# oscarkey/safe-exploration

Measured on AMD Instinct MI355X. Metric: cem_particle_step_evals_per_s, higher is better.
Workload: dtype f64

## Files before the change

### include/sx_amd.h

```cpp
#ifndef SX_AMD_H
#define SX_AMD_H

#include <stdint.h>

#ifdef __cplusplus
extern "C" {
#endif

#define SX_MAX_NS 4
#define SX_MAX_NU 2
#define SX_MAX_D (SX_MAX_NS + SX_MAX_NU)
#define SX_MAX_M 16
#define SX_TILE 16

#define SX_OK 0
#define SX_ERR_ARG 1
#define SX_ERR_UNSUPPORTED 2
#define SX_ERR_LAUNCH 3

#define SX_STATUS_NAN 1
#define SX_STATUS_ZERO_FIX 2
#define SX_STATUS_UB_NONPOS 4

#define SX_OBJ_NEG_VARIANCE 0
// ... 350 lines not shown
int sx_cem_rollout_cons_multi(const sx_gp_model* models, const void* table, const sx_env* env, const sx_con_set* cons,
                              const sx_sat_cost* cost, int E, int P, int H, const double* x0, const double* q0,
                              const double* mean, const double* std, const double* noise, double* actions, double* traj,
                              double* sigma, double* obj_cost, double* con_cost, int32_t* status, void* stream);
int sx_cem_rollout_elites_cons_multi(const sx_gp_model* models, const void* table, const sx_env* env, const sx_con_set* cons,
                                     const sx_sat_cost* cost, int E, int P, int H, const double* x0, const double* q0,
                                     const double* elite_rows, int k, const double* noise, double* actions, double* traj,
                                     double* sigma, double* obj_cost, double* con_cost, int32_t* status, double* mean_out,
                                     double* std_out, void* stream);
int sx_cem_rollout_cons_multi_form(const sx_gp_model* models, int E, int H);

int sx_cem_rollout_starts_cons(const sx_gp_model* model, const sx_env* env, const sx_con_set* cons, int E, int P, int H,
                               const double* mean, const double* std, const double* noise, double* rows, double* traj,
                               double* sigma, double* obj_cost, double* con_cost, int32_t* status, void* stream);

int sx_cem_rollout_starts_multi(const sx_gp_model* models, const void* table, const sx_env* env, int E, int P, int H,
                                const double* mean, const double* std, const double* noise, double* rows, double* traj,
                                double* sigma, double* obj_cost, double* con_cost, int32_t* status , void* stream);
int sx_cem_rollout_starts_cons_multi(const sx_gp_model* models, const void* table, const sx_env* env,
                                     const sx_con_set* cons, int E, int P, int H, const double* mean, const double* std,
                                     const double* noise, double* rows, double* traj, double* sigma, double* obj_cost,
                                     double* con_cost, int32_t* status , void* stream);
int sx_cem_rollout_starts_multi_form(const sx_gp_model* models, int E, int H);

int sx_cem_pack_result(int G, int E, int row_len, const int32_t* status, const int32_t* best_ok, const double* q_block,
                       int64_t q_count, const double* best, double* out, void* stream);

int sx_cem_rank_counts(int E, int P);

int sx_cem_rank_refit(int E, int P, int k, int row_len, const double* con_cost, const double* obj_cost,
                      int64_t cost_stride, const double* actions, int64_t act_stride, int32_t* elite_idx,
                      double* elite_rows, double* mean, double* std, double* best, int32_t* best_ok, void* stream);

#ifdef __cplusplus
}
#endif
#endif
```

### safe_exploration_amd/_lib.py

```python
import ctypes
import os
from ctypes import POINTER, Structure, c_char_p, c_double, c_int, c_int32, c_int64, c_uint8, c_void_p

import numpy as np
import torch

SX_MAX_NS = 4
SX_MAX_NU = 2
SX_MAX_D = SX_MAX_NS + SX_MAX_NU
SX_MAX_M = 16
SX_SAT_MAX_DIM = SX_MAX_NS + 1
SX_TILE = 16
SX_GP_FIT_ENTRY_BYTES = 360
SX_GP_APPEND_ENTRY_BYTES = 408
SX_FEAT_MAX_WIDTH = 32
SX_FEAT_MAX_LAYERS = 3
SX_MLP_MAX_HIDDEN = 4
SX_MLP_MAX_WIDTH = 64

SX_OK, SX_ERR_ARG, SX_ERR_UNSUPPORTED, SX_ERR_LAUNCH = 0, 1, 2, 3
SX_STATUS_NAN, SX_STATUS_ZERO_FIX, SX_STATUS_UB_NONPOS, SX_STATUS_NOT_PD = 1, 2, 4, 8
SX_OBJ_NEG_VARIANCE, SX_OBJ_AFFINE_ABS = 0, 1
SX_CON_TERMINAL, SX_CON_ALL_STATES = 0, 1
SX_PROF_ROLLOUT_FUSED, SX_PROF_RANK, SX_PROF_KSTAR_BIG, SX_PROF_TRMM_BIG, SX_PROF_STEP_BIG, SX_PROF_ROLLOUT_FEAT, SX_PROF_ROLLOUT_MLP = range(7)
# ... 154 lines not shown
                                         c_int] + [c_void_p] * 12),
    'sx_cem_rollout_elites_sat_multi': (c_int, [POINTER(SxGpModel), c_void_p, POINTER(SxEnv), POINTER(SxSatCost), c_int,
                                                c_int, c_int, c_void_p, c_void_p, c_void_p, c_int] + [c_void_p] * 10),
    'sx_cem_rollout_sat_form': (c_int, [POINTER(SxGpModel), c_int]),
    'sx_conset_eval': (c_int, [POINTER(SxEnv), POINTER(SxConSet), c_int] + [c_void_p] * 4 + [c_int, c_void_p, c_void_p]),
    'sx_cem_rollout_cons': (c_int, [POINTER(SxGpModel), POINTER(SxEnv), POINTER(SxConSet), POINTER(SxSatCost), c_int, c_int,
                                    c_int] + [c_void_p] * 12),
    'sx_cem_rollout_elites_cons': (c_int, [POINTER(SxGpModel), POINTER(SxEnv), POINTER(SxConSet), POINTER(SxSatCost), c_int,
                                           c_int, c_int, c_void_p, c_void_p, c_void_p, c_int] + [c_void_p] * 10),
    'sx_cem_rollout_cons_form': (c_int, [POINTER(SxGpModel), c_int]),
    'sx_cem_rollout_cons_multi': (c_int, [POINTER(SxGpModel), c_void_p, POINTER(SxEnv), POINTER(SxConSet),
                                          POINTER(SxSatCost), c_int, c_int, c_int] + [c_void_p] * 12),
    'sx_cem_rollout_elites_cons_multi': (c_int, [POINTER(SxGpModel), c_void_p, POINTER(SxEnv), POINTER(SxConSet),
                                                 POINTER(SxSatCost), c_int, c_int, c_int, c_void_p, c_void_p, c_void_p,
                                                 c_int] + [c_void_p] * 10),
    'sx_cem_rollout_cons_multi_form': (c_int, [POINTER(SxGpModel), c_int, c_int]),
    'sx_cem_rollout_starts_cons': (c_int, [POINTER(SxGpModel), POINTER(SxEnv), POINTER(SxConSet), c_int, c_int, c_int]
                                   + [c_void_p] * 10),
    'sx_cem_rollout_starts_multi': (c_int, [POINTER(SxGpModel), c_void_p, POINTER(SxEnv), c_int, c_int, c_int]
                                    + [c_void_p] * 10),
    'sx_cem_rollout_starts_cons_multi': (c_int, [POINTER(SxGpModel), c_void_p, POINTER(SxEnv), POINTER(SxConSet), c_int,
                                                 c_int, c_int] + [c_void_p] * 10),
    'sx_cem_rollout_starts_multi_form': (c_int, [POINTER(SxGpModel), c_int, c_int]),
    'sx_profile_enable': (c_int, [c_int]),
    'sx_profile_stride': (c_int, [c_int]),
    'sx_profile_stride_kind': (c_int, [c_int, c_int]),
    'sx_profile_collect': (c_int, [c_int, POINTER(c_double), POINTER(c_int64)]),
    'sx_profile_disable': (c_int, []),
    'sx_cem_rank_counts': (c_int, [c_int, c_int]),
    'sx_cem_rollout_form': (c_int, [POINTER(SxGpModel), c_int]),
    'sx_cem_pack_result': (c_int, [c_int, c_int, c_int, c_void_p, c_void_p, c_void_p, c_int64, c_void_p, c_void_p, c_void_p]),
    'sx_cem_rank_refit': (c_int, [c_int, c_int, c_int, c_int, c_void_p, c_void_p, c_int64, c_void_p, c_int64]
                          + [c_void_p] * 7),
}

LIB_PATH = os.environ.get('SX_LIB') or os.path.join(os.path.dirname(os.path.abspath(__file__)), 'csrc', 'libsxamd.so')
_lib = None


class SxError(RuntimeError):
    pass


def lib():
    global _lib
    if _lib is None:
        if not os.path.exists(LIB_PATH):
            raise SxError(f'{LIB_PATH} is missing: build it with `python -c "import __graft_entry__ as g; g.build()"` '
                          f'(safe_exploration_amd has no CPU fallback)')
        handle = ctypes.CDLL(LIB_PATH)
        for name, (res, args) in SIGNATURES.items():
            fn = getattr(handle, name)
            fn.restype = res
            fn.argtypes = args
        _lib = handle
    return _lib


def check(code: int, what: str) -> None:
    if code != SX_OK:
        raise SxError(f'{what}: {_ERR.get(code, code)}')


def ptr(t):
    if t is None:
        return None
# ... 31 lines not shown
```

### safe_exploration_amd/cem_mpc.py

```python
import ctypes
from dataclasses import dataclass
from typing import List, NamedTuple, Optional, Sequence, Tuple

import torch
from torch import Tensor

from . import _lib, distributed
from .costs import SaturatingCost
from .gp_reachability_pytorch import raise_for_status, save_failure_state
from .ssm_cem.gp_ssm_cem import GpCemSSM


@dataclass
class Rollouts:
    trajectories: Optional[Tensor]
    actions: Tensor
    objective_costs: Tensor
    constraint_costs: Tensor
    perf_trajectories: Optional[Tensor] = None
    perf_sigma: Optional[Tensor] = None
    perf_cov: Optional[Tensor] = None


def _rollout(suffix: str, head: tuple, x0: Tensor, horizon: int, n_s: int, n_u: int, words: int, unsupported, *,
             actions, mean, std, noise, q0, want_traj, want_sigma, status, elite_rows, want_dist, workspace=()):
    dev = x0.device
    E = x0.size(0)
    if noise is not None:
        P = noise.size(1)
        actions = torch.empty((E, P, horizon, n_u), dtype=torch.float64, device=dev)
    else:
        P = actions.size(1)
        actions = actions.contiguous()
# ... 732 lines not shown
        raise ValueError(f'{share} particles per GPU rank in {chunks} chunks: num_elites={num_elites} is '
                         f'too large for it (limit {min(share // chunks, RANK_MAX_CANDIDATES // chunks)})')


def expand_init_std(init_std, horizon: int, n_u: int) -> Tensor:
    std = torch.as_tensor(init_std, dtype=torch.float64).cpu()
    return (std.reshape(horizon, -1) if std.dim() > 0 else std).expand(horizon, n_u).clone()


def cem_rank_refit_any(con: Tensor, obj: Tensor, actions: Tensor, k: int, **kw):
    E, P = con.shape
    C = rank_chunks(P)
    if C == 1:
        return cem_rank_refit(con, obj, actions, k, **kw)
    Pc, L = P // C, actions[0, 0].numel()
    if k > Pc or C * k > RANK_MAX_CANDIDATES:
        raise ValueError(f'{P} candidates rank in {C} chunks of {Pc}: k={k} must not exceed the chunk size, nor '
                         f'{C} k the kernel\'s {RANK_MAX_CANDIDATES}')
    local = cem_rank_refit(con.reshape(E * C, Pc), obj.reshape(E * C, Pc), actions.reshape(E * C, Pc, L), k,
                           want_rows=True, want_refit=False)
    flat = local['elite_rows'].reshape(-1)
    return cem_rank_refit(flat, flat[1:], flat[2:], k, cost_stride=2 + L, act_stride=2 + L, row_len=L,
                          num_candidates=C * k, num_problems=E, **kw)


def _hand_off(owner, best: Tensor, best_ok: Tensor, status: Tensor, q_block: Optional[Tensor]):
    G, E, L = status.numel(), best_ok.numel(), best[0].numel()
    n = G + E + 1 + E * L
    packed = torch.empty(n, dtype=torch.float64, device=best.device)
    _lib.check(_lib.lib().sx_cem_pack_result(G, E, L, _lib.ptr(status), _lib.ptr(best_ok), _lib.ptr(q_block),
                                             q_block.numel() if q_block is not None else 0,
                                             _lib.ptr(best.contiguous()), _lib.ptr(packed),
                                             _lib.stream_ptr(best.device)), 'sx_cem_pack_result')
    host = getattr(owner, '_pinned', None)
    if host is None or host.numel() < n:
        owner._pinned = host = torch.empty(max(n, 256), dtype=torch.float64).pin_memory()
    host[:n].copy_(packed, non_blocking=True)
    torch.cuda.current_stream(best.device).synchronize()
    out = host[:n].clone()
    return (out[:G].to(torch.int64), out[G:G + E] != 0, bool(out[G + E] != 0),
            out[G + E + 1:].view(best.shape))


def fold_status(words) -> int:
    out = 0
    for w in words.reshape(-1).tolist():
        out |= int(w)
    return out


def _cem_iterations(iterations: int, rollout, rank, mean: Tensor, std: Tensor):
    rows = out = None
    for it in range(iterations):
        out = rank(it, rollout(it, mean, std, rows))
        if out['mean'] is None:
            rows = out['elite_rows']
        else:
            mean, std = out['mean'].view(mean.shape), out['std'].view(std.shape)
    return out


def _check_solve(owner, x0: Tensor, q_block: Optional[Tensor], best: Tensor, best_ok: Tensor, status: Tensor, where: str,
                 problems):
    words, found, is_nonpoint, best_host = _hand_off(owner, best, best_ok, status, q_block)
    if is_nonpoint:
        raise NotImplementedError(f'{where} starts from point states (all-zero Q), as CemSafeMPC.get_action does')
    statuses = [fold_status(words[r]) for _, r in problems]
    both = _lib.SX_STATUS_NAN | _lib.SX_STATUS_ZERO_FIX
    repeated = False
    for i, (s, r) in enumerate(problems):
        if (statuses[i] & both) == both and owner._last_noise is not None:
            owner.stepwise_fallbacks += 1
            repeated = True
            b, ok, _, st = s.solve(x0[r], noise=owner._last_noise[:, r].contiguous(), stepwise=True)
            w, found[r], _, best_host[r] = _hand_off(owner, b, ok, st, None)
            statuses[i] = fold_status(w)
    for (s, _), st in zip(problems, statuses):
        s.last_status = st
    for i, ((s, r), st) in enumerate(zip(problems, statuses)):
        raise_for_status(st, where if len(problems) == 1 else f'{where} (problem {i})',
                         dump=lambda s=s, r=r: save_failure_state(s._ssm, x0[r], s._last_actions if s is owner else None))
    return best_host, found, repeated


def _checked_cost(cost, n_s: int, kind: Optional[str], on_safety: bool = False):
    if cost is None:
        return None
    if not isinstance(cost, SaturatingCost):
        raise TypeError(f'cost must be a costs.SaturatingCost or None, got {type(cost).__name__}')
    if kind != 'taylor' and not on_safety:
        raise ValueError("a SaturatingCost prices (mean, covariance) pairs: it needs a performance trajectory with "
                         "cem_perf_type='taylor' (perf_type='taylor', n_perf > 0), not "
                         + ('no performance trajectory' if kind is None else f'the {kind!r} form')
                         + ('; without one, cost_on_safety=True (cem_cost_on_safety) prices the safety ellipsoids'
                            if kind is None else ''))
    if cost.n_s != n_s:
        raise ValueError(f'the cost is built for n_s = {cost.n_s}, the model has n_s = {n_s}')
    return cost


class FusedCemMpc:

    def __init__(self, ssm: GpCemSSM, env: _lib.SxEnv, time_horizon: int, num_rollouts: int, num_elites: int,
                 num_iterations: int, *, device=None, seed: int = 0, init_std=1.0, warm_start: str = 'zero',
                 record_rollouts: bool = False, process_group=None, force_exchange: bool = False, n_perf: int = 0,
                 perf_r: int = 1, perf_variance: bool = False, perf_type: str = 'mean_equivalent',
                 perf_terminal_safety: bool = False, cost_on_safety: bool = False, con_set=None):
        self._ssm = ssm
        self._con_set = _checked_con_set(con_set, ssm)
        if con_set is not None:
            if int(n_perf) > 0:
                raise NotImplementedError(f'con_set constrains the safety trajectory of a solve without a performance '
                                          f'trajectory: got n_perf={n_perf} (cem_n_perf > 0 is not built)')
            if process_group is not None:
                raise NotImplementedError('con_set is not built for sharded particles (a process group)')
        self._cost_on_safety = bool(cost_on_safety)
        if self._cost_on_safety and int(n_perf) > 0:
            raise ValueError(f'cost_on_safety=True prices the safety trajectory, which carries the objective only without a '
                             f'performance trajectory: got n_perf={n_perf}.  The cost belongs to one trajectory, chosen by '
                             f"n_perf (n_perf > 0 with perf_type='taylor' prices the performance trajectory)")
        self._env = env
        self._horizon = time_horizon
        self._perf = PerfSpec(n_perf, perf_r, perf_variance, perf_type, perf_terminal_safety).checked(time_horizon)
        if self._perf.on:
            _require_exact_rbf([ssm], 'the performance trajectory is')
            if process_group is not None:
                raise NotImplementedError('the performance trajectory is not built for sharded particles (a process group)')
            self._check_perf_objective(env)
        self.last_perf_actions = None
        self._num_iterations = num_iterations
        self._record = record_rollouts
# ... 121 lines not shown
                           init_std: Optional[Tensor] = None) -> Tuple[Tensor, Tensor]:
        perf = self._perf
        E, dev, H, n_u = x0.size(0), x0.device, perf.row_steps(self._horizon), self._ssm.num_actions
        if init_mean is not None:
            mean = init_mean.to(dev).reshape(E, H, n_u).clone()
        elif self._warm_start == 'safe_policy' and perf.on:
            plan = self.safe_policy_plan(x0, max(self._horizon, perf.n_perf))
            mean = torch.cat([plan[:, :self._horizon], plan[:, perf.r:perf.n_perf]], dim=1).contiguous()
        elif self._warm_start == 'safe_policy':
            mean = self.safe_policy_plan(x0).contiguous()
        else:
            mean = self._constant('zero_mean', E, dev, lambda: torch.zeros((E, H, n_u), dtype=torch.float64, device=dev))
        std = (init_std.to(dev).reshape(E, H, n_u).clone() if init_std is not None else
               self._constant('init_std', E, dev, lambda: self._init_std.to(dev).expand(E, H, n_u).contiguous()))
        return mean, std

    def _refit_in_prologue(self, episodes: int) -> bool:
        chunks = rank_chunks(self._local_rollouts)
        candidates = (self._world * (self._local_elites + (1 if episodes == 1 else 0)) if self._sharded
                      else chunks * self._num_elites if chunks > 1 else self._local_rollouts)
        return fused_refit_applies(self._ssm, episodes, self._local_rollouts, self._horizon, candidates)

    def _rollout_stepwise(self, x0: Tensor, mean: Tensor, std: Tensor, eps: Tensor, status: Tensor):
        acts = (mean.unsqueeze(1) + std.unsqueeze(1) * eps).contiguous()
        cost = self._safety_cost
        per_e = [cem_rollout_stepwise(self._ssm, self._env, x0[e], acts[e], status=status,
                                      group=self._group if self._world > 1 else None,
                                      objective_hook=self._objective_hook if cost is None else None,
                                      **({} if cost is None else dict(cost=cost)),
                                      **_con_set_kw(getattr(self, '_con_set', None))) for e in range(x0.size(0))]
        return dict(actions=acts, traj=None, obj_cost=torch.stack([q['obj_cost'] for q in per_e]),
                    con_cost=torch.stack([q['con_cost'] for q in per_e]))

    def solve(self, x0: Tensor, noise: Optional[Tensor] = None, init_mean: Optional[Tensor] = None,
              init_std: Optional[Tensor] = None, stepwise: bool = False) -> Tuple[Tensor, Tensor, List[Rollouts], Tensor]:
        n_u, H, E, dev = self._ssm.num_actions, self._horizon, x0.size(0), x0.device
        spec = self._perf
        perf, rows_steps = spec.on, spec.row_steps(H)
        L = rows_steps * n_u
        mean, std = self.start_distribution(x0, init_mean, init_std)
        status = self._fresh_status(dev)
        history: List[Rollouts] = []
        xch = None
        stepwise = stepwise or self._always_stepwise
        if noise is None and 'sample_noise' not in vars(self):
            noise = self._next_noise(E)
        self._last_noise, self._last_actions = noise, None
        in_prologue = (not stepwise) and (not perf) and self._refit_in_prologue(E)
        safety_cost = self._safety_cost
        cost_kw = dict({} if safety_cost is None else dict(cost=safety_cost), **_con_set_kw(getattr(self, '_con_set', None)))
        want_traj = self._record or (self._objective_hook is not None and not perf and safety_cost is None)
        if perf and noise is not None:
            noise_safe, noise_tail = noise[:, :, :, :H].contiguous(), noise[:, :, :, H:].contiguous()

        def rollout(it, mean, std, rows):
            nonlocal stepwise, in_prologue
            eps = noise[it] if noise is not None else self.sample_noise(E)
            if noise is None:
                self._last_noise = None
            if self.rollout_events is not None:
                ev = (torch.cuda.Event(enable_timing=True), torch.cuda.Event(enable_timing=True))
                ev[0].record(torch.cuda.current_stream(dev))
            if perf:
                full_mean, full_std = mean, std
                mean, std = mean[:, :H].contiguous(), std[:, :H].contiguous()
                eps, eps_tail = ((noise_safe[it], noise_tail[it]) if noise is not None
                                 else (eps[:, :, :H].contiguous(), eps[:, :, H:].contiguous()))
            if stepwise:
                r = self._rollout_stepwise(x0, mean, std, eps, status)
            else:
                try:
                    r = cem_rollout(self._ssm, self._env, x0, H, mean=mean, std=std, elite_rows=rows,
                                    noise=eps.contiguous(), want_traj=want_traj, status=status, **cost_kw)
                except FusedJunkUnsupported:
                    if it != 0:
                        raise
                    stepwise, in_prologue = True, False
                    r = self._rollout_stepwise(x0, mean, std, eps, status)
            if perf:
                hook, n_s = (self._objective_hook if self._cost is None else None), self._ssm.num_states
# ... 32 lines not shown
            self._exchanges_seen += 1
            if timed:
                xev = [torch.cuda.Event(enable_timing=True) for _ in range(4)]
                xev[0].record(torch.cuda.current_stream(dev))
            if E == 1:
                cem_rank_refit_any(r['con_cost'], r['obj_cost'], r['actions'], k, want_refit=False,
                                   rows_out=xch.local_slot(it))
            else:
                local = cem_rank_refit_any(r['con_cost'], r['obj_cost'], r['actions'], k, want_rows=True, want_refit=False)
                xch.local_slot(it).copy_(local['elite_rows'])
            last = it == self._num_iterations - 1
            if timed:
                xev[1].record(torch.cuda.current_stream(dev))
            cand, words = xch.exchange(it, status if last else None)
            if timed:
                xev[2].record(torch.cuda.current_stream(dev))
            if last:
                status = words
            flat = cand.reshape(-1)
            out = cem_rank_refit(flat, flat[1:], flat[2:], self._num_elites, cost_stride=2 + L,
                                 act_stride=2 + L, row_len=L, num_candidates=xch.candidates, num_problems=E,
                                 want_rows=in_prologue, want_refit=not in_prologue)
            if timed:
                xev[3].record(torch.cuda.current_stream(dev))
                self.exchange_events.append(xev)
            return out

        out = _cem_iterations(self._num_iterations, rollout, rank, mean, std)
        return out['best'].view(E, rows_steps, n_u), out['best_ok'], history, status

    def _solve_checked(self, x0: Tensor, where: str, q_block: Optional[Tensor] = None):
        if q_block is not None and not q_block.is_contiguous():
            q_block = q_block.contiguous()
        best, best_ok, history, status = self.solve(x0)
        best_host, found, repeated = _check_solve(self, x0, q_block, best, best_ok, status, where, [(self, slice(None))])
        if self._perf.on:
            self.last_perf_actions = best_host[:, self._horizon:]
            best_host = best_host[:, :self._horizon]
        return best_host, found, [] if repeated else history

    def get_actions_batch(self, states: Tensor) -> Tuple[Tensor, Tensor, List[Rollouts]]:
        x0, q_block = split_flat_states(states, self._ssm.num_states, self._device)
        return self._solve_checked(x0, 'get_actions_batch', q_block=q_block)

    def get_actions(self, state: Tensor) -> Tuple[Optional[Tensor], List[Rollouts]]:
        x0, q_block = split_flat_states(state.reshape(1, -1), self._ssm.num_states, self._device, episodes=1)
        best, found, history = self._solve_checked(x0, 'get_actions', q_block=q_block)
        if not bool(found[0]):
            return None, history
        return best[0], history


class SharedPolicy(NamedTuple):
    what: str
    con_set: str = 'none'
    exact_rbf: bool = False
    label: str = ''


def _setting(solver, attr):
    v = attr(solver) if callable(attr) else getattr(solver, attr, None)
    if isinstance(v, Tensor):
        return tuple(v.reshape(-1).tolist()), False
    return (bytes(v), False) if isinstance(v, ctypes.Structure) else (v, True)


def _model_shape(solver) -> tuple:
    return solver._ssm.num_states, solver._ssm.num_actions
# ... 825 lines not shown
```

### safe_exploration_amd/csrc/sx_gp_rollout.hip

```cpp
#include <hip/hip_runtime.h>

#include <cstdlib>
#include <cstring>
#include <vector>

#include "../../include/sx_amd.h"
#include "sx_big.hpp"
#include "sx_big_launch.hpp"
#include "sx_host.hpp"
#include "sx_launch.hpp"
#include "sx_rw_launch.hpp"
#include "sx_stream_launch.hpp"

namespace sx {

#ifdef SX_STAMPS
extern unsigned long long* g_stamp_host;
#endif

struct RolloutPlan {
    int form;
    bool ok;
    size_t lds;
    int nrb;
};

struct FormOverride {
    int form;
    bool strict;
    bool refuses() const { return strict && form >= 0; }
};
static const FormOverride& form_override() {
    static const FormOverride o = [] {
        const char* e = std::getenv("SX_ROLLOUT");
        const int form = !e                            ? -1
                         : std::strcmp(e, "stream") == 0 ? SX_FORM_STREAM
                         : std::strcmp(e, "rw") == 0     ? SX_FORM_RW
                         : std::strcmp(e, "rh") == 0     ? SX_FORM_RH
                                                         : -1;
        return FormOverride{form, std::getenv("SX_ROLLOUT_STRICT") != nullptr};
    }();
    return o;
}

template <int NS, int NU>
static int resident_lds_bytes(int n_train, int n_pad, int H, size_t* rh, size_t* rw) {
    *rh = rollout_rh_lds_bytes<NS, NU>(n_train, n_pad, H);
    *rw = rollout_rw_lds_bytes<NS, NU>(n_train, n_pad, H);
    return SX_OK;
}
static int resident_lds_bytes(int ns, int nu, int n_train, int n_pad, int H, size_t* rh, size_t* rw) {
#define CALL(NS, NU) resident_lds_bytes<NS, NU>(n_train, n_pad, H, rh, rw)
    SX_DISPATCH(ns, nu, CALL);
#undef CALL
}

static bool elite_rows_fit(int ns, int nu, int H) { return 2 * H * nu <= 256 + 256 * ns; }

static RolloutPlan plan_rollout(const sx_gp_model* m, int sh, int H, bool elites) {
    const int ns = m->n_s, nu = m->n_u - sh, n_train = m->n_train, n_pad = m->n_pad;
    const StreamPlan s = plan_stream(ns, nu, sh, n_train, n_pad, H);
    bool ok = rollout_compiled(ns, nu, sh);
    if (s.form < 0) return {SX_FORM_BIG, ok && sh == 0 && !elites, 0, 0};
    if (elites && !elite_rows_fit(ns, nu, H)) ok = false;
    if (s.form == SX_FORM_BYOUT) return {SX_FORM_BYOUT, ok, s.lds, 0};
    const RolloutPlan stream{SX_FORM_STREAM, ok, s.lds, 0};
    const FormOverride& o = form_override();
    if (!ok || sh > 0 || o.form == SX_FORM_STREAM) return stream;
    size_t rh, rw;
    resident_lds_bytes(ns, nu, n_train, n_pad, H, &rh, &rw);
    if (o.form != SX_FORM_RW && rh <= kMaxLdsBytes) return {SX_FORM_RH, true, rh, n_pad >> 4};
    if (o.form != SX_FORM_RH && rw <= kMaxLdsBytes) return {SX_FORM_RW, true, rw, n_pad >> 4};
    return {SX_FORM_STREAM, !o.refuses(), stream.lds, 0};
}

template <int NS, int NU, int SH>
static int launch_rollout(const sx_gp_model* m, const sx_env* env, const RolloutPtrs& rp, double* workspace,
                          int64_t workspace_bytes, hipStream_t stream) {
    RolloutPlan plan = plan_rollout(m, SH, rp.H, rp.elite_rows != nullptr);
    if (!plan.ok) return SX_ERR_UNSUPPORTED;
    if constexpr (SH == 0) {
        if (plan.form == SX_FORM_BIG) return launch_rollout_big<NS, NU>(m, env, rp, workspace, workspace_bytes, stream);
    }
    ReachConst<NS, NU> rc;
    CostConst<SX_MAX_M, NS, NU> cc;
    if (int r = env_consts<NS, NU>(env, rc, cc)) return r;
    RolloutPtrs rps = rp;
#ifdef SX_STAMPS
    rps.stamps = g_stamp_host;
#endif
    if constexpr (SH == 0) {
        if (plan.form == SX_FORM_RH || plan.form == SX_FORM_RW) {
            const int r = plan.form == SX_FORM_RH
                              ? launch_rollout_rh<NS, NU>(make_gp_const<NS, NU>(m, 8), rc, cc, rps, plan.nrb, plan.lds, stream)
                              : launch_rollout_rw<NS, NU>(make_gp_const<NS, NU>(m, kRwWaves), rc, cc, rps, plan.nrb, plan.lds,
                                                          stream);
            if (r != SX_ERR_UNSUPPORTED || form_override().refuses()) return r;
            plan = {SX_FORM_STREAM, true, rollout_stream_lds_bytes(NS, NU, SH, m->n_train, m->n_pad, rp.H, false), 0};
        }
    }
    return launch_stream<StreamPlain<SH>, NS, NU>(make_gp_const<NS, NU + SH>(m, kRolloutThreads / 64), rc, cc, rps, nullptr,
                                                  plan.form == SX_FORM_BYOUT, plan.lds, stream);
}

template <class V, int NS, int NU>
static int stream_rollout(const sx_gp_model* models, const void* table, const sx_env* env, const sx_sat_cost* cost,
                          const sx_con_set* cons, const double* gains, const RolloutPtrs& rp, hipStream_t stream) {
    const StreamPlan plan = plan_stream_multi(models, V::MM ? rp.E : 1, rp.H);
    if (plan.form < 0 || (rp.elite_rows && !elite_rows_fit(NS, NU, rp.H))) return SX_ERR_UNSUPPORTED;
    ReachConst<NS, NU> rc;
    CostConst<SX_MAX_M, NS, NU> cc;
    if constexpr (V::KF) {
// ... 44 lines not shown
    std::vector<GpConst<NS, NS + NU>> host(E);
    for (int i = 0; i < E; ++i) host[i] = make_gp_const<NS, NU>(&models[i], kRolloutThreads / 64);
    return copy_model_table(host, table, stream);
}

static RolloutPtrs with_elites(RolloutPtrs rp, const double* elite_rows, int k, double* mean_out, double* std_out) {
    rp.elite_rows = elite_rows;
    rp.elite_k = k;
    rp.mean_out = mean_out;
    rp.std_out = std_out;
    return rp;
}

struct Objective {
    bool sat;
    const sx_sat_cost* cost;
};
constexpr Objective kEnvObjective{false, nullptr};

static bool rollout_shapes_ok(const sx_gp_model* model, const sx_env* env, int query_shift) {
    return model->n_s == env->n_s && query_shift >= 0 && query_shift <= env->n_u && model->n_u == env->n_u + query_shift;
}

static bool multi_models_ok(const sx_gp_model* models, int E) {
    if (!models || E <= 0) return false;
    const int ns = models[0].n_s, nu = models[0].n_u;
    if (ns <= 0 || ns > SX_MAX_NS || nu <= 0 || nu > SX_MAX_NU) return false;
    for (int i = 0; i < E; ++i)
        if (models[i].n_s != ns || models[i].n_u != nu || models[i].n_train <= 0 || models[i].n_pad <= 0) return false;
    return true;
}

static int cem_rollout_single(const sx_gp_model* model, const sx_env* env, int query_shift, Objective obj, bool elites,
                              const RolloutPtrs& rp, void* workspace, int64_t workspace_bytes, void* stream) {
    if (!model || (elites && !rp.elite_rows) || !rollout_args_ok(env, rp) || !rollout_shapes_ok(model, env, query_shift))
        return SX_ERR_ARG;
    if (obj.sat) {
        if (!sat_cost_ok(obj.cost, env->n_s)) return SX_ERR_ARG;
        return stream_dispatch<StreamSat<false>>(model, nullptr, env, obj.cost, rp, stream);
    }
#define CALL(NS, NU, SH) launch_rollout<NS, NU, SH>(model, env, rp, (double*)workspace, workspace_bytes, (hipStream_t)stream)
    SX_ROLLOUT_DISPATCH(env->n_s, env->n_u, query_shift, CALL);
#undef CALL
}

static int cem_rollout_cons(const sx_gp_model* model, const sx_env* env, const sx_con_set* cons, const sx_sat_cost* cost,
                            bool elites, const RolloutPtrs& rp, void* stream) {
    if (!model || (elites && !rp.elite_rows) || !rollout_args_ok(env, rp) || !rollout_shapes_ok(model, env, 0))
        return SX_ERR_ARG;
    if (!con_set_ok(cons, env->n_s) || (cost && !sat_cost_ok(cost, env->n_s))) return SX_ERR_ARG;
    if (cost) return stream_dispatch<StreamCons<true>>(model, nullptr, env, cost, rp, stream, cons);
    return stream_dispatch<StreamCons<false>>(model, nullptr, env, nullptr, rp, stream, cons);
}

static int cem_rollout_cons_multi(const sx_gp_model* models, const void* table, const sx_env* env, const sx_con_set* cons,
                                  const sx_sat_cost* cost, bool elites, const RolloutPtrs& rp, void* stream) {
    if (!table || (elites && !rp.elite_rows) || !rollout_args_ok(env, rp) || !multi_models_ok(models, rp.E)) return SX_ERR_ARG;
    if (models[0].n_s != env->n_s || models[0].n_u != env->n_u) return SX_ERR_ARG;
    if (!con_set_ok(cons, env->n_s) || (cost && !sat_cost_ok(cost, env->n_s))) return SX_ERR_ARG;
    if (cost) return stream_dispatch<StreamCons<true, true>>(models, table, env, cost, rp, stream, cons);
    return stream_dispatch<StreamCons<false, true>>(models, table, env, nullptr, rp, stream, cons);
}

static int cem_rollout_multi(const sx_gp_model* models, const void* table, const sx_env* env, Objective obj, bool elites,
                             const RolloutPtrs& rp, void* stream) {
    if (!table || (elites && !rp.elite_rows) || !rollout_args_ok(env, rp) || !multi_models_ok(models, rp.E)) return SX_ERR_ARG;
    if (models[0].n_s != env->n_s || models[0].n_u != env->n_u) return SX_ERR_ARG;
    if (!obj.sat) return stream_dispatch<StreamPlain<0, true>>(models, table, env, nullptr, rp, stream);
    if (!sat_cost_ok(obj.cost, env->n_s)) return SX_ERR_ARG;
    return stream_dispatch<StreamSat<true>>(models, table, env, obj.cost, rp, stream);
}

static int stream_form(const sx_gp_model* models, int E, int H) {
    return models && H > 0 ? plan_stream_multi(models, E, H).form : -1;
}

// ... 228 lines not shown
```

### safe_exploration_amd/csrc/sx_rank.hip

```cpp
#include <hip/hip_runtime.h>

#include <atomic>
#include <cstdlib>
#include <map>
#include <mutex>

#include "../../include/sx_amd.h"
#include "sx_launch.hpp"
#include "sx_rank.hpp"
#include "sx_rank_count.hpp"

#ifdef SX_STAMPS
namespace sx {
unsigned long long* g_stamp_host = nullptr;
}

extern "C" int sx_debug_set_stamps(unsigned long long* dev_buf) {
    sx::g_stamp_host = dev_buf;
    return hipMemcpyToSymbol(HIP_SYMBOL(sx::g_stamp_buf), &dev_buf, sizeof(dev_buf)) == hipSuccess ? SX_OK : SX_ERR_LAUNCH;
}
#endif

extern "C" {

namespace sx {
__global__ __launch_bounds__(256) void pack_result_kernel(int G, int E, int L, const int* __restrict__ status,
                                                          const int* __restrict__ best_ok, const double* __restrict__ q_block,
                                                          long long q_count, const double* __restrict__ best,
                                                          double* __restrict__ out) {
    __shared__ int any_nz;
    const int tid = threadIdx.x;
    if (tid == 0) any_nz = 0;
    __syncthreads();
    int nz = 0;
    if (q_block)
        for (long long i = tid; i < q_count; i += blockDim.x) nz |= (q_block[i] != 0.0) ? 1 : 0;
    if (nz) atomicOr(&any_nz, 1);
    for (int i = tid; i < G; i += blockDim.x) out[i] = (double)status[i];
    for (int i = tid; i < E; i += blockDim.x) out[G + i] = (double)best_ok[i];
    for (int i = tid; i < E * L; i += blockDim.x) out[G + E + 1 + i] = best[i];
    __syncthreads();
    if (tid == 0) out[G + E] = any_nz ? 1.0 : 0.0;
}
}

int sx_cem_pack_result(int G, int E, int row_len, const int32_t* status, const int32_t* best_ok, const double* q_block,
                       int64_t q_count, const double* best, double* out, void* stream) {
    if (G <= 0 || E <= 0 || row_len <= 0 || !status || !best_ok || !best || !out || q_count < 0) return SX_ERR_ARG;
    hipLaunchKernelGGL(sx::pack_result_kernel, dim3(1), dim3(256), 0, (hipStream_t)stream, G, E, row_len, status, best_ok,
                       q_count > 0 ? q_block : nullptr, (long long)q_count, best, out);
    return sx::check_launch();
}

int sx_cem_rank_counts(int E, int P) {
    if (E <= 0 || P <= 0 || P > sx::kCountMaxP || E > sx::kCountMaxE) return 0;
    static const char* const forced = std::getenv("SX_RANK_PATH");
    if (forced && forced[0] == 's') return 0;
    if (forced && forced[0] == 'c') return 1;
    return (long long)E * ((P + 15) / 16) <= sx::kCountMaxGrid ? 1 : 0;
}

int sx_cem_rank_refit(int E, int P, int k, int row_len, const double* con_cost, const double* obj_cost,
                      int64_t cost_stride, const double* actions, int64_t act_stride, int32_t* elite_idx,
                      double* elite_rows, double* mean, double* std, double* best, int32_t* best_ok, void* stream) {
    if (!con_cost || !obj_cost || !actions || E <= 0 || P <= 0 || k <= 0 || row_len <= 0) return SX_ERR_ARG;
    if (k > P) return SX_ERR_ARG;
    if (k > sx::kRankMaxK) return SX_ERR_UNSUPPORTED;
    sx::RankArgs ra{P,      k,          row_len,    con_cost, obj_cost, (long long)cost_stride,
                    actions, (long long)act_stride, elite_idx, elite_rows, mean,     std,
                    best,   best_ok};
    const bool count = sx_cem_rank_counts(E, P) != 0 && (elite_rows || !mean);
    const int tiles = (P + 15) / 16;
    if (count) {
        const size_t lds = (size_t)((P + 127) & ~127) * sizeof(sx::CountKey);
        if (int rc = sx::allow_lds(sx::cem_rank_count_kernel, lds)) return rc;
        static std::atomic<unsigned int> seq{0};
        unsigned int* tickets = nullptr;
        if (mean) {
            static std::mutex mu;
            static std::map<int, unsigned int*> base;
            int dev = 0;
            (void)hipGetDevice(&dev);
            std::lock_guard<std::mutex> lock(mu);
            auto it = base.find(dev);
            if (it == base.end()) {
                unsigned int* p = nullptr;
                if (hipGetSymbolAddress((void**)&p, HIP_SYMBOL(sx::g_rank_tickets)) != hipSuccess) return SX_ERR_LAUNCH;
                it = base.emplace(dev, p).first;
            }
            tickets = it->second + (size_t)(seq.fetch_add(1) % sx::kCountTicketSlots) * sx::kCountMaxE;
        }
        sx::launch(SX_PROF_RANK, sx::cem_rank_count_kernel, dim3((unsigned)tiles, (unsigned)E), dim3(sx::kCountThreads), lds,
                   (hipStream_t)stream, ra, tickets);
        return sx::check_launch();
    }
    if (P > sx::kRankThreads * sx::kRankSlots) return SX_ERR_UNSUPPORTED;
    const int slots = (P + sx::kRankThreads - 1) / sx::kRankThreads;
    if (slots <= 4)
        sx::launch(SX_PROF_RANK, sx::cem_rank_kernel<4>, dim3(E), dim3(sx::kRankThreads), 0, (hipStream_t)stream, ra);
    else if (slots <= 8)
        sx::launch(SX_PROF_RANK, sx::cem_rank_kernel<8>, dim3(E), dim3(sx::kRankThreads), 0, (hipStream_t)stream, ra);
    else
        sx::launch(SX_PROF_RANK, sx::cem_rank_kernel<sx::kRankSlots>, dim3(E), dim3(sx::kRankThreads), 0, (hipStream_t)stream, ra);
    return sx::check_launch();
}

}
```

Baseline: 469.2 million.

## Add native C++ CEM solve loop to bypass per-iteration Python dispatch

Adds a native sx_cem_solve entry point that plans the rollout and rank paths once, lays out one cached workspace, and runs all CEM iterations (rollout, rank/refit, and optional result packing plus async device-to-host copy) from C++. The Python solver routes to this path when none of a long list of refusal conditions apply, cutting per-iteration Python/ctypes overhead, tensor allocations and the separate hand-off launch. The cost is a second code path that must stay consistent with the Python one. It also relies on many guard rules to fall back correctly.

```diff
diff --git a/include/sx_amd.h b/include/sx_amd.h
--- a/include/sx_amd.h
+++ b/include/sx_amd.h
@@ -406,6 +406,14 @@
                       int64_t cost_stride, const double* actions, int64_t act_stride, int32_t* elite_idx,
                       double* elite_rows, double* mean, double* std, double* best, int32_t* best_ok, void* stream);
 
+int64_t sx_cem_solve_workspace_bytes(const sx_gp_model* model, const sx_env* env, int E, int P, int H, int k,
+                                     int iterations);
+
+int sx_cem_solve(const sx_gp_model* model, const sx_env* env, int E, int P, int H, int k, int iterations, const double* x0,
+                 const double* mean0, const double* std0, const double* noise, void* workspace, int64_t workspace_bytes,
+                 int32_t* status, double* best_out, int32_t* best_ok_out, double* pack_out_host, const double* q_block,
+                 int64_t q_count, void* stream);
+
 #ifdef __cplusplus
 }
 #endif
diff --git a/safe_exploration_amd/_lib.py b/safe_exploration_amd/_lib.py
--- a/safe_exploration_amd/_lib.py
+++ b/safe_exploration_amd/_lib.py
@@ -210,6 +210,9 @@
     'sx_cem_pack_result': (c_int, [c_int, c_int, c_int, c_void_p, c_void_p, c_void_p, c_int64, c_void_p, c_void_p, c_void_p]),
     'sx_cem_rank_refit': (c_int, [c_int, c_int, c_int, c_int, c_void_p, c_void_p, c_int64, c_void_p, c_int64]
                           + [c_void_p] * 7),
+    'sx_cem_solve_workspace_bytes': (c_int64, [POINTER(SxGpModel), POINTER(SxEnv), c_int, c_int, c_int, c_int, c_int]),
+    'sx_cem_solve': (c_int, [POINTER(SxGpModel), POINTER(SxEnv), c_int, c_int, c_int, c_int, c_int] + [c_void_p] * 5
+                     + [c_int64] + [c_void_p] * 5 + [c_int64, c_void_p]),
 }
 
 LIB_PATH = os.environ.get('SX_LIB') or os.path.join(os.path.dirname(os.path.abspath(__file__)), 'csrc', 'libsxamd.so')
diff --git a/safe_exploration_amd/cem_mpc.py b/safe_exploration_amd/cem_mpc.py
--- a/safe_exploration_amd/cem_mpc.py
+++ b/safe_exploration_amd/cem_mpc.py
@@ -1,4 +1,5 @@
 import ctypes
+import os
 from dataclasses import dataclass
 from typing import List, NamedTuple, Optional, Sequence, Tuple
 
@@ -797,14 +798,24 @@
                                              q_block.numel() if q_block is not None else 0,
                                              _lib.ptr(best.contiguous()), _lib.ptr(packed),
                                              _lib.stream_ptr(best.device)), 'sx_cem_pack_result')
+    host = _pinned_buffer(owner, n)
+    host[:n].copy_(packed, non_blocking=True)
+    torch.cuda.current_stream(best.device).synchronize()
+    return _read_packed(host, G, E, best.shape)
+
+
+def _pinned_buffer(owner, n: int) -> Tensor:
     host = getattr(owner, '_pinned', None)
     if host is None or host.numel() < n:
         owner._pinned = host = torch.empty(max(n, 256), dtype=torch.float64).pin_memory()
-    host[:n].copy_(packed, non_blocking=True)
-    torch.cuda.current_stream(best.device).synchronize()
+    return host
+
+
+def _read_packed(host: Tensor, G: int, E: int, shape):
+    n = G + E + 1 + torch.Size(shape).numel()
     out = host[:n].clone()
     return (out[:G].to(torch.int64), out[G:G + E] != 0, bool(out[G + E] != 0),
-            out[G + E + 1:].view(best.shape))
+            out[G + E + 1:].view(shape))
 
 
 def fold_status(words) -> int:
@@ -826,8 +837,8 @@
 
 
 def _check_solve(owner, x0: Tensor, q_block: Optional[Tensor], best: Tensor, best_ok: Tensor, status: Tensor, where: str,
-                 problems):
-    words, found, is_nonpoint, best_host = _hand_off(owner, best, best_ok, status, q_block)
+                 problems, handed=None):
+    words, found, is_nonpoint, best_host = handed if handed is not None else _hand_off(owner, best, best_ok, status, q_block)
     if is_nonpoint:
         raise NotImplementedError(f'{where} starts from point states (all-zero Q), as CemSafeMPC.get_action does')
     statuses = [fold_status(words[r]) for _, r in problems]
@@ -862,6 +873,34 @@
     if cost.n_s != n_s:
         raise ValueError(f'the cost is built for n_s = {cost.n_s}, the model has n_s = {n_s}')
     return cost
+
+
+def native_solve_refusal(solver, x0: Tensor, stepwise: bool = False) -> Optional[str]:
+    get = lambda name, default=None: getattr(solver, name, default)
+    rules = [
+        (os.environ.get('SX_NATIVE_SOLVE', '1') == '0', 'SX_NATIVE_SOLVE=0'),
+        (not x0.is_cuda or get('_env') is None, 'no device solve (host tensors or no environment)'),
+        (get('_sharded', False), 'sharded particles or force_exchange'),
+        (stepwise or get('_always_stepwise', False), 'the step-by-step rollout'),
+        (get('_objective_hook') is not None, 'an objective hook'),
+        (get('_record', False), 'recorded rollouts'),
+        ('sample_noise' in vars(solver), 'a patched sample_noise'),
+        (perf_spec_of(solver).on, 'a performance trajectory'),
+        (get('_cost_on_safety', False), 'cost_on_safety'),
+        (get('_con_set') is not None, 'a constraint set (con_set)'),
+        (get('rollout_events') is not None, 'events around every rollout launch'),
+        (getattr(get('_ssm'), 'kernel_family', 'rbf') != 'rbf', 'a junk-dimension, feature-GP, MC-dropout or step-by-step model'),
+        (rank_chunks(get('_local_rollouts', 1)) > 1, 'two-level ranking'),
+        (any(globals()[name] is not fn for name, fn in _LOOP_WRAPPERS.items()), 'a replaced rollout or ranking wrapper'),
+        (not isinstance(_lib.lib(), ctypes.CDLL), 'a replaced library handle'),
+    ]
+    for refused, why in rules:
+        if refused:
+            return why
+    return None
+
+
+_LOOP_WRAPPERS = {'cem_rollout': cem_rollout, 'cem_rank_refit_any': cem_rank_refit_any, 'cem_rank_refit': cem_rank_refit}
 
 
 class FusedCemMpc:
@@ -1049,6 +1088,53 @@
         return dict(actions=acts, traj=None, obj_cost=torch.stack([q['obj_cost'] for q in per_e]),
                     con_cost=torch.stack([q['con_cost'] for q in per_e]))
 
+    def _native_plan(self, E: int, dev):
+        model, env = self._ssm.device_model, self._env
+        key = (model.n_train, model.n_pad, self._local_rollouts, self._horizon, self._num_elites, self._num_iterations, dev)
+        cache = self.__dict__.setdefault('_native', {})
+        plan = cache.get(E)
+        if plan is None or plan[0] is not model or plan[1] is not env or plan[2] != key:
+            head = (ctypes.byref(model), ctypes.byref(env), E, self._local_rollouts, self._horizon, self._num_elites,
+                    self._num_iterations)
+            nbytes = int(_lib.lib().sx_cem_solve_workspace_bytes(*head))
+            if nbytes < 0:
+                raise _lib.SxError('sx_cem_solve_workspace_bytes: bad arguments')
+            old = plan[3] if plan is not None else None
+            ws = None
+            if nbytes > 0:
+                ws = old[1] if old is not None and old[2] == nbytes and old[1].device == dev else \
+                    torch.empty((nbytes + 7) // 8, dtype=torch.float64, device=dev)
+            cache[E] = plan = (model, env, key, (head, ws, nbytes) if nbytes > 0 else None)
+        return plan[3]
+
+    def _solve_native(self, x0: Tensor, mean: Tensor, std: Tensor, noise: Tensor, status: Tensor):
+        E, dev, H, n_u, P = x0.size(0), x0.device, self._horizon, self._ssm.num_actions, self._local_rollouts
+        plan = self._native_plan(E, dev)
+        if plan is None or tuple(noise.shape) != (self._num_iterations, E, P, H, n_u):
+            return None
+        _lib.require_gpu(x0, 'x0')
+        head, ws, nbytes = plan
+        L = H * n_u
+        best = torch.empty((E, H, n_u), dtype=torch.float64, device=dev)
+        best_ok = torch.empty((E,), dtype=torch.int32, device=dev)
+        request, host, q_block = self.__dict__.pop('_hand_off_request', None), None, None
+        if request is not None:
+            q_block = request[0]
+            host = _pinned_buffer(self, 1 + E + 1 + E * L)
+        code = _lib.lib().sx_cem_solve(*head, _lib.ptr(x0.contiguous()), _lib.ptr(mean.contiguous()),
+                                       _lib.ptr(std.contiguous()), _lib.ptr(noise.contiguous()), _lib.ptr(ws), nbytes,
+                                       _lib.ptr(status), _lib.ptr(best), _lib.ptr(best_ok),
+                                       None if host is None else ctypes.c_void_p(host.data_ptr()), _lib.ptr(q_block),
+                                       q_block.numel() if q_block is not None else 0, _lib.stream_ptr(dev))
+        if code == _lib.SX_ERR_UNSUPPORTED:
+            return None
+        _lib.check(code, 'sx_cem_solve')
+        per_iter = E * P * (L + 2)
+        self._last_actions = ws[(self._num_iterations - 1) * per_iter:][:E * P * L].view(E, P, H, n_u)
+        if host is not None:
+            self._handed_off = (host, best, best_ok, status)
+        return best, best_ok, [], status
+
     def solve(self, x0: Tensor, noise: Optional[Tensor] = None, init_mean: Optional[Tensor] = None,
               init_std: Optional[Tensor] = None, stepwise: bool = False) -> Tuple[Tensor, Tensor, List[Rollouts], Tensor]:
         n_u, H, E, dev = self._ssm.num_actions, self._horizon, x0.size(0), x0.device
@@ -1063,6 +1149,10 @@
         if noise is None and 'sample_noise' not in vars(self):
             noise = self._next_noise(E)
         self._last_noise, self._last_actions = noise, None
+        if noise is not None and native_solve_refusal(self, x0, stepwise) is None:
+            out = self._solve_native(x0, mean, std, noise, status)
+            if out is not None:
+                return out
         in_prologue = (not stepwise) and (not perf) and self._refit_in_prologue(E)
         safety_cost = self._safety_cost
         cost_kw = dict({} if safety_cost is None else dict(cost=safety_cost), **_con_set_kw(getattr(self, '_con_set', None)))
@@ -1161,8 +1251,19 @@
     def _solve_checked(self, x0: Tensor, where: str, q_block: Optional[Tensor] = None):
         if q_block is not None and not q_block.is_contiguous():
             q_block = q_block.contiguous()
-        best, best_ok, history, status = self.solve(x0)
-        best_host, found, repeated = _check_solve(self, x0, q_block, best, best_ok, status, where, [(self, slice(None))])
+        self._hand_off_request, self._handed_off = (q_block,), None
+        try:
+            best, best_ok, history, status = self.solve(x0)
+        finally:
+            self._hand_off_request = None
+        handed, self._handed_off = self._handed_off, None
+        if handed is not None and (handed[1] is best and handed[2] is best_ok and handed[3] is status):
+            torch.cuda.current_stream(best.device).synchronize()
+            handed = _read_packed(handed[0], status.numel(), best_ok.numel(), best.shape)
+        else:
+            handed = None
+        best_host, found, repeated = _check_solve(self, x0, q_block, best, best_ok, status, where, [(self, slice(None))],
+                                                  handed=handed)
         if self._perf.on:
             self.last_perf_actions = best_host[:, self._horizon:]
             best_host = best_host[:, :self._horizon]
diff --git a/safe_exploration_amd/csrc/sx_gp_rollout.hip b/safe_exploration_amd/csrc/sx_gp_rollout.hip
--- a/safe_exploration_amd/csrc/sx_gp_rollout.hip
+++ b/safe_exploration_amd/csrc/sx_gp_rollout.hip
@@ -10,6 +10,7 @@
 #include "sx_host.hpp"
 #include "sx_launch.hpp"
 #include "sx_rw_launch.hpp"
+#include "sx_solve.hpp"
 #include "sx_stream_launch.hpp"
 
 namespace sx {
@@ -18,12 +19,6 @@
 extern unsigned long long* g_stamp_host;
 #endif
 
-struct RolloutPlan {
-    int form;
-    bool ok;
-    size_t lds;
-    int nrb;
-};
 
 struct FormOverride {
     int form;
@@ -55,9 +50,7 @@
 #undef CALL
 }
 
-static bool elite_rows_fit(int ns, int nu, int H) { return 2 * H * nu <= 256 + 256 * ns; }
-
-static RolloutPlan plan_rollout(const sx_gp_model* m, int sh, int H, bool elites) {
+RolloutPlan plan_rollout(const sx_gp_model* m, int sh, int H, bool elites) {
     const int ns = m->n_s, nu = m->n_u - sh, n_train = m->n_train, n_pad = m->n_pad;
     const StreamPlan s = plan_stream(ns, nu, sh, n_train, n_pad, H);
     bool ok = rollout_compiled(ns, nu, sh);
@@ -76,8 +69,8 @@
 
 template <int NS, int NU, int SH>
 static int launch_rollout(const sx_gp_model* m, const sx_env* env, const RolloutPtrs& rp, double* workspace,
-                          int64_t workspace_bytes, hipStream_t stream) {
-    RolloutPlan plan = plan_rollout(m, SH, rp.H, rp.elite_rows != nullptr);
+                          int64_t workspace_bytes, hipStream_t stream, const RolloutPlan* planned) {
+    RolloutPlan plan = planned ? *planned : plan_rollout(m, SH, rp.H, rp.elite_rows != nullptr);
     if (!plan.ok) return SX_ERR_UNSUPPORTED;
     if constexpr (SH == 0) {
         if (plan.form == SX_FORM_BIG) return launch_rollout_big<NS, NU>(m, env, rp, workspace, workspace_bytes, stream);
@@ -188,16 +181,23 @@
 }
 
 static int cem_rollout_single(const sx_gp_model* model, const sx_env* env, int query_shift, Objective obj, bool elites,
-                              const RolloutPtrs& rp, void* workspace, int64_t workspace_bytes, void* stream) {
+                              const RolloutPtrs& rp, void* workspace, int64_t workspace_bytes, void* stream,
+                              const RolloutPlan* planned = nullptr) {
     if (!model || (elites && !rp.elite_rows) || !rollout_args_ok(env, rp) || !rollout_shapes_ok(model, env, query_shift))
         return SX_ERR_ARG;
     if (obj.sat) {
         if (!sat_cost_ok(obj.cost, env->n_s)) return SX_ERR_ARG;
         return stream_dispatch<StreamSat<false>>(model, nullptr, env, obj.cost, rp, stream);
     }
-#define CALL(NS, NU, SH) launch_rollout<NS, NU, SH>(model, env, rp, (double*)workspace, workspace_bytes, (hipStream_t)stream)
+#define CALL(NS, NU, SH) \
+    launch_rollout<NS, NU, SH>(model, env, rp, (double*)workspace, workspace_bytes, (hipStream_t)stream, planned)
     SX_ROLLOUT_DISPATCH(env->n_s, env->n_u, query_shift, CALL);
 #undef CALL
+}
+
+int cem_rollout_planned(const sx_gp_model* model, const sx_env* env, const RolloutPlan& plan, const RolloutPtrs& rp,
+                        void* stream) {
+    return cem_rollout_single(model, env, 0, kEnvObjective, rp.elite_rows != nullptr, rp, nullptr, 0, stream, &plan);
 }
 
 static int cem_rollout_cons(const sx_gp_model* model, const sx_env* env, const sx_con_set* cons, const sx_sat_cost* cost,
diff --git a/safe_exploration_amd/csrc/sx_rank.hip b/safe_exploration_amd/csrc/sx_rank.hip
--- a/safe_exploration_amd/csrc/sx_rank.hip
+++ b/safe_exploration_amd/csrc/sx_rank.hip
@@ -9,6 +9,7 @@
 #include "sx_launch.hpp"
 #include "sx_rank.hpp"
 #include "sx_rank_count.hpp"
+#include "sx_solve.hpp"
 
 #ifdef SX_STAMPS
 namespace sx {
@@ -47,9 +48,7 @@
 int sx_cem_pack_result(int G, int E, int row_len, const int32_t* status, const int32_t* best_ok, const double* q_block,
                        int64_t q_count, const double* best, double* out, void* stream) {
     if (G <= 0 || E <= 0 || row_len <= 0 || !status || !best_ok || !best || !out || q_count < 0) return SX_ERR_ARG;
-    hipLaunchKernelGGL(sx::pack_result_kernel, dim3(1), dim3(256), 0, (hipStream_t)stream, G, E, row_len, status, best_ok,
-                       q_count > 0 ? q_block : nullptr, (long long)q_count, best, out);
-    return sx::check_launch();
+    return sx::cem_pack_result(G, E, row_len, status, best_ok, q_block, q_count, best, out, (hipStream_t)stream);
 }
 
 int sx_cem_rank_counts(int E, int P) {
@@ -65,13 +64,37 @@
                       double* elite_rows, double* mean, double* std, double* best, int32_t* best_ok, void* stream) {
     if (!con_cost || !obj_cost || !actions || E <= 0 || P <= 0 || k <= 0 || row_len <= 0) return SX_ERR_ARG;
     if (k > P) return SX_ERR_ARG;
-    if (k > sx::kRankMaxK) return SX_ERR_UNSUPPORTED;
+    const int path = sx::rank_path(E, P, k, elite_rows != nullptr, mean != nullptr);
+    if (path < 0) return -path;
+    return sx::cem_rank_refit(path, E, P, k, row_len, con_cost, obj_cost, cost_stride, actions, act_stride, elite_idx,
+                              elite_rows, mean, std, best, best_ok, (hipStream_t)stream);
+}
+
+}
+
+namespace sx {
+
+int cem_pack_result(int G, int E, int row_len, const int32_t* status, const int32_t* best_ok, const double* q_block,
+                    int64_t q_count, const double* best, double* out, hipStream_t stream) {
+    hipLaunchKernelGGL(pack_result_kernel, dim3(1), dim3(256), 0, stream, G, E, row_len, status, best_ok,
+                       q_count > 0 ? q_block : nullptr, (long long)q_count, best, out);
+    return check_launch();
+}
+
+int rank_path(int E, int P, int k, bool want_rows, bool want_refit) {
+    if (k > kRankMaxK) return -SX_ERR_UNSUPPORTED;
+    if (sx_cem_rank_counts(E, P) != 0 && (want_rows || !want_refit)) return 1;
+    return P > kRankThreads * kRankSlots ? -SX_ERR_UNSUPPORTED : 0;
+}
+
+int cem_rank_refit(int path, int E, int P, int k, int row_len, const double* con_cost, const double* obj_cost,
+                   int64_t cost_stride, const double* actions, int64_t act_stride, int32_t* elite_idx, double* elite_rows,
+                   double* mean, double* std, double* best, int32_t* best_ok, hipStream_t stream) {
     sx::RankArgs ra{P,      k,          row_len,    con_cost, obj_cost, (long long)cost_stride,
                     actions, (long long)act_stride, elite_idx, elite_rows, mean,     std,
                     best,   best_ok};
-    const bool count = sx_cem_rank_counts(E, P) != 0 && (elite_rows || !mean);
     const int tiles = (P + 15) / 16;
-    if (count) {
+    if (path == 1) {
         const size_t lds = (size_t)((P + 127) & ~127) * sizeof(sx::CountKey);
         if (int rc = sx::allow_lds(sx::cem_rank_count_kernel, lds)) return rc;
         static std::atomic<unsigned int> seq{0};
@@ -94,7 +117,6 @@
                    (hipStream_t)stream, ra, tickets);
         return sx::check_launch();
     }
-    if (P > sx::kRankThreads * sx::kRankSlots) return SX_ERR_UNSUPPORTED;
     const int slots = (P + sx::kRankThreads - 1) / sx::kRankThreads;
     if (slots <= 4)
         sx::launch(SX_PROF_RANK, sx::cem_rank_kernel<4>, dim3(E), dim3(sx::kRankThreads), 0, (hipStream_t)stream, ra);
diff --git a/safe_exploration_amd/csrc/sx_solve.hip b/safe_exploration_amd/csrc/sx_solve.hip
--- /dev/null
+++ b/safe_exploration_amd/csrc/sx_solve.hip
@@ -0,0 +1,132 @@
+#include <hip/hip_runtime.h>
+
+#include "../../include/sx_amd.h"
+#include "sx_rollout.hpp"
+#include "sx_solve.hpp"
+
+namespace sx {
+
+struct SolveLayout {
+    int64_t per_iter;
+    int64_t obj, con;
+    int64_t rows[2];
+    int64_t mean[2], std[2];
+    int64_t best;
+    int64_t packed;
+    int64_t idx_bytes, ok_bytes;
+    int64_t bytes;
+};
+
+struct SolvePlan {
+    bool ok;
+    bool in_prologue;
+    RolloutPlan first, later;
+    int rank;
+    SolveLayout lay;
+};
+
+static SolveLayout layout_solve(int E, int P, int L, int k, int iterations) {
+    SolveLayout l{};
+    const int64_t EP = (int64_t)E * P, EL = (int64_t)E * L, rows = (int64_t)E * k * (2 + L);
+    l.obj = EP * L;
+    l.con = l.obj + EP;
+    l.per_iter = l.con + EP;
+    int64_t at = l.per_iter * iterations;
+    auto take = [&at](int64_t n) {
+        const int64_t here = at;
+        at += n;
+        return here;
+    };
+    for (int b = 0; b < 2; ++b) l.rows[b] = take(rows);
+    for (int b = 0; b < 2; ++b) {
+        l.mean[b] = take(EL);
+        l.std[b] = take(EL);
+    }
+    l.best = take(EL);
+    l.packed = take(1 + E + 1 + EL);
+    l.idx_bytes = at * (int64_t)sizeof(double);
+    l.ok_bytes = l.idx_bytes + (int64_t)E * k * (int64_t)sizeof(int32_t);
+    l.bytes = l.ok_bytes + (int64_t)E * (int64_t)sizeof(int32_t);
+    return l;
+}
+
+static SolvePlan plan_solve(const sx_gp_model* m, const sx_env* env, int E, int P, int H, int k, int iterations) {
+    SolvePlan p{};
+    const int ns = m->n_s, nu = m->n_u;
+    if (ns != env->n_s || nu != env->n_u || ns <= 0 || ns > SX_MAX_NS || nu <= 0 || nu > SX_MAX_NU) return p;
+    if (m->n_train <= 0 || m->n_pad <= 0 || env->m <= 0 || env->m > SX_MAX_M || k > P) return p;
+    p.first = plan_rollout(m, 0, H, false);
+    if (!p.first.ok || p.first.form == SX_FORM_BIG) return p;
+    p.in_prologue = elite_rows_fit(ns, nu, H) && sx_cem_rank_counts(E, P) == 1;
+    p.later = p.in_prologue && iterations > 1 ? plan_rollout(m, 0, H, true) : p.first;
+    if (!p.later.ok || p.later.form == SX_FORM_BIG) return p;
+    p.rank = rank_path(E, P, k, p.in_prologue, !p.in_prologue);
+    if (p.rank < 0) return p;
+    p.lay = layout_solve(E, P, H * nu, k, iterations);
+    p.ok = true;
+    return p;
+}
+
+}
+
+extern "C" {
+
+int64_t sx_cem_solve_workspace_bytes(const sx_gp_model* model, const sx_env* env, int E, int P, int H, int k,
+                                     int iterations) {
+    if (!model || !env || E <= 0 || P <= 0 || H <= 0 || k <= 0 || iterations <= 0) return -1;
+    const sx::SolvePlan plan = sx::plan_solve(model, env, E, P, H, k, iterations);
+    return plan.ok ? plan.lay.bytes : 0;
+}
+
+int sx_cem_solve(const sx_gp_model* model, const sx_env* env, int E, int P, int H, int k, int iterations, const double* x0,
+                 const double* mean0, const double* std0, const double* noise, void* workspace, int64_t workspace_bytes,
+                 int32_t* status, double* best_out, int32_t* best_ok_out, double* pack_out_host, const double* q_block,
+                 int64_t q_count, void* stream) {
+    if (!model || !env || !x0 || !mean0 || !std0 || !noise || !workspace || !status || !best_out || !best_ok_out)
+        return SX_ERR_ARG;
+    if (E <= 0 || P <= 0 || H <= 0 || k <= 0 || iterations <= 0 || q_count < 0) return SX_ERR_ARG;
+    const sx::SolvePlan plan = sx::plan_solve(model, env, E, P, H, k, iterations);
+    if (!plan.ok) return SX_ERR_UNSUPPORTED;
+    const sx::SolveLayout& l = plan.lay;
+    if (workspace_bytes < l.bytes) return SX_ERR_ARG;
+
+    const int L = H * model->n_u;
+    double* const ws = static_cast<double*>(workspace);
+    int32_t* const idx = reinterpret_cast<int32_t*>(static_cast<char*>(workspace) + l.idx_bytes);
+    int32_t* const ok_ws = reinterpret_cast<int32_t*>(static_cast<char*>(workspace) + l.ok_bytes);
+    const int64_t noise_iter = (int64_t)E * P * L;
+    hipStream_t s = (hipStream_t)stream;
+    for (int it = 0; it < iterations; ++it) {
+        double* const iter = ws + l.per_iter * it;
+        double *const actions = iter, *const obj = iter + l.obj, *const con = iter + l.con;
+        const bool elites = plan.in_prologue && it > 0;
+        sx::RolloutPtrs rp{x0, nullptr, nullptr, nullptr, noise + noise_iter * it, actions, nullptr, nullptr, obj, con,
+                           status, E, P, H};
+        if (elites) {
+            rp.elite_rows = ws + l.rows[(it - 1) & 1];
+            rp.elite_k = k;
+        } else {
+            rp.mean = it == 0 ? mean0 : ws + l.mean[(it - 1) & 1];
+            rp.std = it == 0 ? std0 : ws + l.std[(it - 1) & 1];
+        }
+        if (int rc = sx::cem_rollout_planned(model, env, elites ? plan.later : plan.first, rp, stream)) return rc;
+        const bool last = it == iterations - 1;
+        const int b = it & 1;
+        if (int rc = sx::cem_rank_refit(plan.rank, E, P, k, L, con, obj, 1, actions, L, idx,
+                                        plan.in_prologue ? ws + l.rows[b] : nullptr,
+                                        plan.in_prologue ? nullptr : ws + l.mean[b],
+                                        plan.in_prologue ? nullptr : ws + l.std[b], last ? best_out : ws + l.best,
+                                        last ? best_ok_out : ok_ws, s))
+            return rc;
+    }
+    if (pack_out_host) {
+        double* const packed = ws + l.packed;
+        if (int rc = sx::cem_pack_result(1, E, L, status, best_ok_out, q_block, q_block ? q_count : 0, best_out, packed, s))
+            return rc;
+        const size_t n = (size_t)(1 + E + 1 + (int64_t)E * L) * sizeof(double);
+        if (hipMemcpyAsync(pack_out_host, packed, n, hipMemcpyDeviceToHost, s) != hipSuccess) return SX_ERR_LAUNCH;
+    }
+    return SX_OK;
+}
+
+}
diff --git a/safe_exploration_amd/csrc/sx_solve.hpp b/safe_exploration_amd/csrc/sx_solve.hpp
--- /dev/null
+++ b/safe_exploration_amd/csrc/sx_solve.hpp
@@ -0,0 +1,35 @@
+#pragma once
+#include <hip/hip_runtime.h>
+
+#include <cstdint>
+
+#include "../../include/sx_amd.h"
+
+namespace sx {
+
+struct RolloutPtrs;
+
+struct RolloutPlan {
+    int form;
+    bool ok;
+    size_t lds;
+    int nrb;
+};
+
+RolloutPlan plan_rollout(const sx_gp_model* m, int sh, int H, bool elites);
+
+inline bool elite_rows_fit(int ns, int nu, int H) { return 2 * H * nu <= 256 + 256 * ns; }
+
+int cem_rollout_planned(const sx_gp_model* model, const sx_env* env, const RolloutPlan& plan, const RolloutPtrs& rp,
+                        void* stream);
+
+int rank_path(int E, int P, int k, bool want_rows, bool want_refit);
+
+int cem_rank_refit(int path, int E, int P, int k, int row_len, const double* con_cost, const double* obj_cost,
+                   int64_t cost_stride, const double* actions, int64_t act_stride, int32_t* elite_idx, double* elite_rows,
+                   double* mean, double* std, double* best, int32_t* best_ok, hipStream_t stream);
+
+int cem_pack_result(int G, int E, int row_len, const int32_t* status, const int32_t* best_ok, const double* q_block,
+                    int64_t q_count, const double* best, double* out, hipStream_t stream);
+
+}
```

New measurement: 468.8 million (median of 2 runs). No clear change (-0.1%).
